# Coder-Yu/QRec

Hardware: NVIDIA H100
Metric: BPR triples/sec at d=64 (higher is better)
Workload: dtype f32

## Files before the change

include/qrec.h:

```cpp
#ifndef QREC_H_
#define QREC_H_

#include <stdint.h>

#ifdef __cplusplus
extern "C" {
#endif

#define QREC_OK 0
#define QREC_ERR_ARG (-1)
#define QREC_ERR_CUDA (-2)
#define QREC_ERR_STATE (-3)
#define QREC_ERR_NOMEM (-4)

const char* qrec_last_error(void);
const char* qrec_version(void);
int64_t qrec_launch_count(void);

typedef struct qrec_mt19937 {
  uint32_t mt[624];
  uint32_t index;
} qrec_mt19937;

int qrec_mt_seed(qrec_mt19937* st, uint64_t seed);
// ... 78 lines not shown

int qrec_bpr_sgd_batch_tma_f32(float* dev_P, float* dev_Q, int32_t d, int64_t n,
                               const int32_t* dev_u, const int32_t* dev_i, const int32_t* dev_j,
                               float lr, float reg_u, float reg_i, double* dev_loss, void* stream);

int qrec_bpr_sgd_usermajor_f32(float* dev_P, float* dev_Q, int32_t d, int32_t n_users, int64_t n, int32_t num_items,
                               const int64_t* dev_rowptr, const int32_t* dev_i, const int32_t* dev_j,
                               float lr, float reg_u, float reg_i, double* dev_loss, void* stream);

int qrec_bpr_epoch_usermajor_f32(float* dev_P, float* dev_Q, int32_t d, int32_t n_users, int64_t n,
                                 const int64_t* dev_rowptr, const int32_t* dev_i,
                                 const int64_t* dev_rated_rowptr, const int32_t* dev_rated_cols,
                                 int32_t num_items, uint64_t seed, uint32_t epoch, int32_t* dev_j_out,
                                 float lr, float reg_u, float reg_i, double* dev_loss, void* stream);

int qrec_rated_signature_build(int32_t n_users, const int64_t* dev_rated_rowptr, const int32_t* dev_rated_cols,
                               uint32_t* dev_sig, void* stream);
int qrec_bpr_epoch_usermajor_sig_f32(float* dev_P, float* dev_Q, int32_t d, int32_t n_users, int64_t n,
                                     const int64_t* dev_rowptr, const int32_t* dev_i,
                                     const int64_t* dev_rated_rowptr, const int32_t* dev_rated_cols,
                                     const uint32_t* dev_rated_sig, int32_t num_items, uint64_t seed,
                                     uint32_t epoch, int32_t* dev_j_out, float lr, float reg_u, float reg_i,
                                     double* dev_loss, void* stream);

int qrec_bpr_sgd_staged_f32(float* dev_P, int32_t d, int64_t n, const int32_t* dev_u,
                            const int32_t* dev_pos_i, const int32_t* dev_pos_j, const float* dev_R,
                            float* dev_D, float lr, float reg_u, float reg_i, double* dev_loss,
                            void* stream);

int qrec_sumsq_f32(const float* dev_x, int64_t n, double* dev_out, void* stream);
int qrec_sumsq_f64(const double* dev_x, int64_t n, double* dev_out, void* stream);

int qrec_table_snapshot_f32(const float* dev_src, float* dev_dst, int64_t n, void* stream);

int qrec_table_delta_f32(const float* dev_Q, const float* dev_B, float* dev_D, float* dev_S, int64_t n, void* stream);
int qrec_table_merge_f32(float* dev_Q, float* dev_B, const float* dev_D, const float* dev_S, int64_t n, void* stream);
int qrec_table_reduce_scatter_p2p_f32(const float* const* peer_D, int32_t world, int32_t rank, float* dev_S, int64_t n,
                                      void* stream);
int qrec_table_gather_merge_p2p_f32(const float* const* peer_S, int32_t world, float* dev_Q, float* dev_B,
                                    const float* dev_D, int64_t n, void* stream);

int qrec_score_topn_f32(const float* dev_U, const float* dev_V, int32_t d, int32_t n_items,
                        const int32_t* dev_user_ids, int32_t n_rows, const int64_t* dev_rated_rowptr,
                        const int32_t* dev_rated_cols, float rated_value, int32_t N, int32_t* dev_out_ids,
                        float* dev_out_scores, void* stream);
int qrec_score_topn_tc_f32(const float* dev_U, const float* dev_V, int32_t d, int32_t n_items,
                           const int32_t* dev_user_ids, int32_t n_rows, const int64_t* dev_rated_rowptr,
                           const int32_t* dev_rated_cols, float rated_value, int32_t N, int32_t* dev_out_ids,
                           float* dev_out_scores, void* stream);

int qrec_adj_normalize_f32(int32_t n_rows, const int64_t* dev_rowptr, const int32_t* dev_cols, const int32_t* dev_pair,
                           const float* dev_pair_w, float* dev_deg, float* dev_vals, void* stream);
int qrec_edge_keep_philox(int64_t n_lines, float drop_rate, uint64_t seed, uint32_t tag, uint32_t epoch,
                          uint8_t* dev_keep, void* stream);
int qrec_adj_line_weights_f32(int64_t n_lines, const int32_t* dev_line_pair, const uint8_t* dev_keep, int64_t n_pairs,
                              float* dev_pair_w, void* stream);
int qrec_adj_subgraph_count(int32_t n_rows, const int64_t* dev_rowptr, const int32_t* dev_pair, const float* dev_pair_w,
                            float* dev_deg, int64_t* dev_new_rowptr, int64_t* dev_scan_scratch, void* stream);
int qrec_adj_subgraph_fill_f32(int32_t n_rows, const int64_t* dev_rowptr, const int32_t* dev_cols, const int32_t* dev_pair,
                               const float* dev_pair_w, const float* dev_deg, const int64_t* dev_new_rowptr,
                               int32_t* dev_new_cols, float* dev_new_vals, void* stream);

int qrec_ubench_row_ops_f32(float* dev_table, int64_t rows, int64_t n_ops, int32_t mode, uint32_t seed,
                            float* dev_sink, void* stream);

typedef struct qrec_ctx qrec_ctx;
// ... 274 lines not shown
```

qrec_b200/_lib.py:

```python
import ctypes as C
import os

_HERE = os.path.dirname(os.path.abspath(__file__))
LIB_PATH = os.path.join(_HERE, 'libqrec.so')

c_i32p = C.POINTER(C.c_int32)
c_i64p = C.POINTER(C.c_int64)
c_u32p = C.POINTER(C.c_uint32)
c_u8p = C.POINTER(C.c_uint8)
c_f64p = C.POINTER(C.c_double)
vp = C.c_void_p


class MTState(C.Structure):
    _fields_ = [('mt', C.c_uint32 * 624), ('index', C.c_uint32)]


MTp = C.POINTER(MTState)

SIGNATURES = {
    'qrec_last_error': (C.c_char_p, []),
    'qrec_version': (C.c_char_p, []),
    'qrec_launch_count': (C.c_int64, []),
    'qrec_mt_seed': (C.c_int, [MTp, C.c_uint64]),
# ... 86 lines not shown
                                            vp, vp, vp, vp, C.c_int32, vp]),
    'qrec_svdpp_sgd_ordered_f64': (C.c_int, [vp, vp, vp, vp, vp, C.c_int32, C.c_int64, vp, vp, vp, vp, vp, C.c_double,
                                             C.c_double, C.c_double, C.c_double, C.c_double, C.c_double, vp, vp]),
    'qrec_svdpp_sgd_ordered_f32': (C.c_int, [vp, vp, vp, vp, vp, C.c_int32, C.c_int64, vp, vp, vp, vp, vp, C.c_float,
                                             C.c_float, C.c_float, C.c_float, C.c_float, C.c_float, vp, vp]),
    'qrec_svdpp_epoch_usermajor_f32': (C.c_int, [vp, vp, vp, vp, vp, C.c_int32, C.c_int32, vp, vp, vp, vp, C.c_float,
                                                 C.c_float, C.c_float, C.c_float, C.c_float, C.c_float, vp, C.c_int64,
                                                 vp]),
    'qrec_bpr_sgd_batch_f32': (C.c_int, [vp, vp, C.c_int32, C.c_int64, vp, vp, vp, C.c_float,
                                         C.c_float, C.c_float, vp, vp]),
    'qrec_bpr_sgd_batch_tma_f32': (C.c_int, [vp, vp, C.c_int32, C.c_int64, vp, vp, vp, C.c_float,
                                             C.c_float, C.c_float, vp, vp]),
    'qrec_bpr_sgd_usermajor_f32': (C.c_int, [vp, vp, C.c_int32, C.c_int32, C.c_int64, C.c_int32, vp, vp, vp, C.c_float,
                                             C.c_float, C.c_float, vp, vp]),
    'qrec_bpr_epoch_usermajor_f32': (C.c_int, [vp, vp, C.c_int32, C.c_int32, C.c_int64, vp, vp, vp, vp, C.c_int32,
                                               C.c_uint64, C.c_uint32, vp, C.c_float, C.c_float, C.c_float, vp, vp]),
    'qrec_bpr_sgd_staged_f32': (C.c_int, [vp, C.c_int32, C.c_int64, vp, vp, vp, vp, vp, C.c_float, C.c_float,
                                          C.c_float, vp, vp]),
    'qrec_ubench_row_ops_f32': (C.c_int, [vp, C.c_int64, C.c_int64, C.c_int32, C.c_uint32, vp, vp]),
    'qrec_table_delta_f32': (C.c_int, [vp, vp, vp, vp, C.c_int64, vp]),
    'qrec_table_merge_f32': (C.c_int, [vp, vp, vp, vp, C.c_int64, vp]),
    'qrec_table_reduce_scatter_p2p_f32': (C.c_int, [C.POINTER(vp), C.c_int32, C.c_int32, vp, C.c_int64, vp]),
    'qrec_table_gather_merge_p2p_f32': (C.c_int, [C.POINTER(vp), C.c_int32, vp, vp, vp, C.c_int64, vp]),
    'qrec_score_topn_f32': (C.c_int, [vp, vp, C.c_int32, C.c_int32, vp, C.c_int32, vp, vp, C.c_float, C.c_int32, vp, vp, vp]),
    'qrec_score_topn_tc_f32': (C.c_int, [vp, vp, C.c_int32, C.c_int32, vp, C.c_int32, vp, vp, C.c_float, C.c_int32, vp, vp, vp]),
    'qrec_adj_normalize_f32': (C.c_int, [C.c_int32, vp, vp, vp, vp, vp, vp, vp]),
    'qrec_edge_keep_philox': (C.c_int, [C.c_int64, C.c_float, C.c_uint64, C.c_uint32, C.c_uint32, vp, vp]),
    'qrec_adj_line_weights_f32': (C.c_int, [C.c_int64, vp, vp, C.c_int64, vp, vp]),
    'qrec_adj_subgraph_count': (C.c_int, [C.c_int32, vp, vp, vp, vp, vp, vp, vp]),
    'qrec_adj_subgraph_fill_f32': (C.c_int, [C.c_int32, vp, vp, vp, vp, vp, vp, vp, vp, vp]),
    'qrec_sumsq_f32': (C.c_int, [vp, C.c_int64, vp, vp]),
    'qrec_sumsq_f64': (C.c_int, [vp, C.c_int64, vp, vp]),
    'qrec_table_snapshot_f32': (C.c_int, [vp, vp, C.c_int64, vp]),
    'qrec_ctx_create': (C.c_int, [C.c_int, C.c_int64, C.POINTER(vp)]),
    'qrec_ctx_destroy': (C.c_int, [vp]),
    'qrec_ctx_set_rated_signature': (C.c_int, [vp, vp]),
    'qrec_bpr_epoch_host': (C.c_int, [vp, vp, vp, C.c_int32, C.c_int64, vp, vp, vp, C.c_float,
                                      C.c_float, C.c_float, c_f64p]),
    'qrec_bpr_epoch_usermajor_host': (C.c_int, [vp, vp, vp, C.c_int32, C.c_int32, vp, vp, vp, vp, C.c_int32, C.c_uint64,
                                                C.c_uint32, C.c_float, C.c_float, C.c_float, c_f64p]),
    'qrec_spmm_csr_f32': (C.c_int, [C.c_int32, C.c_int64, vp, vp, vp, vp, vp, C.c_int32, vp, C.c_float, vp]),
    'qrec_spmm_csr_rowsplit_f32': (C.c_int, [C.c_int32, C.c_int64, vp, vp, vp, vp, vp, C.c_int32, vp, C.c_float, vp]),
    'qrec_spmm_csr_scatter_rows_f32': (C.c_int, [C.c_int32, C.c_int32, vp, vp, vp, vp, vp, vp, C.c_int32, vp, C.c_float, vp]),
    'qrec_spmm_csr_rows_f32': (C.c_int, [C.c_int32, vp, vp, vp, vp, vp, vp, C.c_int32, C.c_int32, vp, C.c_float, vp]),
    'qrec_bpr_grad_scatter_f32': (C.c_int, [vp, vp, C.c_int32, C.c_int64, vp, vp, vp, C.c_float,
                                            C.c_float, vp, vp, vp, vp]),
    'qrec_bpr_grad_scatter_scaled_f32': (C.c_int, [vp, vp, C.c_int32, C.c_int64, vp, vp, vp, vp, C.c_float,
                                                   C.c_float, vp, vp, vp, vp]),
    'qrec_bpr_partial_scores_f32': (C.c_int, [vp, vp, C.c_int32, C.c_int64, vp, vp, vp, C.c_float, vp, vp, vp]),
    'qrec_bpr_grad_from_scores_f32': (C.c_int, [vp, vp, C.c_int32, C.c_int64, vp, vp, vp, vp, C.c_float, C.c_float, C.c_float, vp, vp, vp, vp]),
    'qrec_adam_dense_tf1_f32': (C.c_int, [vp, vp, vp, vp, C.c_int64, C.c_float, C.c_float,
                                          C.c_float, C.c_float, C.c_int64, vp]),
    'qrec_adam_dense_tf1_devstep_f32': (C.c_int, [vp, vp, vp, vp, C.c_int64, vp, C.c_float, C.c_float, C.c_float, vp]),
    'qrec_axpby_f32': (C.c_int, [vp, vp, vp, C.c_float, C.c_float, C.c_int64, vp]),
    'qrec_simgcl_perturb_f32': (C.c_int, [vp, C.c_int64, C.c_int32, C.c_int32, C.c_float, C.c_uint64, C.c_uint32,
                                          C.c_uint32, vp, C.c_float, vp]),
    'qrec_simgcl_perturb_rows_f32': (C.c_int, [vp, C.c_int64, C.c_int64, C.c_int32, C.c_int32, C.c_float, C.c_uint64, C.c_uint32,
                                               C.c_uint32, vp, C.c_float, vp]),
    'qrec_simgcl_perturb_listed_f32': (C.c_int, [vp, vp, C.c_int64, C.c_int64, C.c_int32, C.c_int32, C.c_float, C.c_uint64, C.c_uint32,
                                                  C.c_uint32, vp, C.c_float, vp]),
    'qrec_gather_normalize_f32': (C.c_int, [vp, vp, C.c_int32, C.c_int32, vp, vp, vp]),
    'qrec_infonce_rows_f32': (C.c_int, [vp, C.c_int32, C.c_float, vp, vp]),
    'qrec_normalize_bwd_scatter_f32': (C.c_int, [vp, vp, vp, vp, C.c_int32, C.c_int32, C.c_float, vp, vp]),
    'qrec_sgemm_f32': (C.c_int, [C.c_int32, C.c_int32, C.c_int32, C.c_int32, C.c_int32, C.c_float, vp,
                                 C.c_int32, vp, C.c_int32, C.c_float, vp, C.c_int32, vp]),
    'qrec_ngcf_act_fwd_f32': (C.c_int, [vp, C.c_int64, C.c_int32, C.c_float, C.c_int32, C.c_uint64,
# ... 47 lines not shown
```

qrec_b200/csrc/bpr_kernels.cu:

```cuda
#include <cmath>

#include "common.h"
#include "device.cuh"
#include "lane_shape.h"
#include "philox.cuh"
#include "bpr_step.cuh"
#include "um_waves.cuh"

namespace {

using namespace qrec;
using namespace qrec::bpr;

template <typename T, int E>
__global__ void __launch_bounds__(256)
bpr_sgd_ordered_kernel(T* __restrict__ P, T* __restrict__ Q, int d, long long n,
                       const int* __restrict__ u, const int* __restrict__ i,
                       const int* __restrict__ j, const int* __restrict__ wu,
                       const int* __restrict__ wi, const int* __restrict__ wj, int* ver_p,
                       int* ver_q, unsigned long long* ticket, T lr, T reg_u, T reg_i,
                       double* loss) {
  const int lane = threadIdx.x & 31;
  double local_loss = 0.0;
  const T a_u = mul_rn(lr, reg_u), a_i = mul_rn(lr, reg_i);
// ... 233 lines not shown
          float* trip = slot + (size_t)(r * TPW + sub) * ROWS * D;
          if (TMA_MASK & 1) *reinterpret_cast<float4*>(trip + SLOT_P * D + l * 4) = dp;
          else red_add_v4(P + (size_t)uu[r] * D + l * 4, dp);
          if (TMA_MASK & 2) *reinterpret_cast<float4*>(trip + SLOT_I * D + l * 4) = dqi;
          else red_add_v4(Q + (size_t)ii[r] * D + l * 4, dqi);
          if (TMA_MASK & 4) *reinterpret_cast<float4*>(trip + SLOT_J * D + l * 4) = dqj;
          else red_add_v4(Q + (size_t)jj[r] * D + l * 4, dqj);
        }
      }
      asm volatile("fence.proxy.async.shared::cta;" ::: "memory");
      __syncwarp();
      if (l < 3 && ((TMA_MASK >> l) & 1)) {
        const int srow = (l == 0) ? SLOT_P : (l == 1 ? SLOT_I : SLOT_J);
#pragma unroll
        for (int r = 0; r < UNROLL; ++r) {
          if (ok[r]) {
            float* dst = (l == 0) ? (P + (size_t)uu[r] * D) : (Q + (size_t)(l == 1 ? ii[r] : jj[r]) * D);
            const float* src = slot + (size_t)(r * TPW + sub) * ROWS * D + srow * D;
            asm volatile("cp.reduce.async.bulk.global.shared::cta.bulk_group.add.f32 [%0], [%1], %2;" ::"l"(dst),
                         "r"((uint32_t)__cvta_generic_to_shared(src)), "n"(D * 4)
                         : "memory");
          }
        }
        asm volatile("cp.async.bulk.commit_group;" ::: "memory");
      }
      buf ^= 1;
    }
  }
  if (l < 3) asm volatile("cp.async.bulk.wait_group 0;" ::: "memory");
  block_add_loss(lsum, loss);
}


template <int LPR, int G, bool FULL, bool SAMPLE, int MINB = 3, bool SIG = false>
__global__ void __launch_bounds__(256, MINB)
bpr_sgd_usermajor_kernel(float* __restrict__ P, float* __restrict__ Q, const float* __restrict__ Qr, int nvec, long long n,
                         const int* __restrict__ wave_user, const long long* __restrict__ rowptr,
                         const int* __restrict__ i, const int* __restrict__ j, float lr, float reg_u, float reg_i,
                         double* loss, FusedSampler fs, long long trip_off, const uint32_t* __restrict__ rated_sig) {
  constexpr int GPW = 32 / LPR;
  const int lane = threadIdx.x & 31;
  const int sub = lane / LPR, l = lane % LPR;
  const unsigned gmask = (LPR == 32) ? 0xffffffffu : (((1u << LPR) - 1u) << (sub * LPR));
  const int group = (int)((blockIdx.x * blockDim.x + threadIdx.x) >> 5) * GPW + sub;
  const int ngroups = (int)((gridDim.x * blockDim.x) >> 5) * GPW;
  const int d = FULL ? LPR * 4 : nvec * 4;
  const bool act = FULL ? true : (l < nvec);
  const float a_u = lr * reg_u, a_i = lr * reg_i;
  const float one_m_au = 1.0f - a_u, one_m_ai = 1.0f - a_i;
  float lsum = 0.f;
  qrec::pdl_launch_dependents();
  bool waited = false;
  const int ub = __ldg(wave_user + 1);
  for (int uu = __ldg(wave_user) + group; uu < ub; uu += ngroups) {
    long long lo = __ldg(rowptr + uu) - trip_off, hi = __ldg(rowptr + uu + 1) - trip_off;
    lo = lo > 0 ? lo : 0;
    hi = hi < n ? hi : n;
    if (lo >= hi) continue;
    float* prow = P + (size_t)uu * d + l * 4;
    float4 p = act ? *reinterpret_cast<const float4*>(prow) : make_float4(0.f, 0.f, 0.f, 0.f);
    long long rated_lo = 0, rated_hi = 0;
    if (SAMPLE) {
      rated_lo = __ldg(fs.rated_rowptr + uu);
      rated_hi = __ldg(fs.rated_rowptr + uu + 1);
    }
    for (long long base = lo; base < hi; base += LPR) {
      const int m = (hi - base) < LPR ? (int)(hi - base) : LPR;
      int mj = 0, mi = 0;
      if (l < m) {
        mi = __ldg(i + base + l);
        if (SAMPLE) {
          if (SIG)
            mj = qrec::sample_negative_sig(base + l + trip_off, fs.epoch, fs.seed_lo, fs.seed_hi, fs.num_items,
                                           fs.rated_cols, rated_lo, rated_hi,
                                           rated_sig + (size_t)uu * qrec::RATED_SIG_WORDS);
          else
            mj = qrec::sample_negative(base + l + trip_off, fs.epoch, fs.seed_lo, fs.seed_hi, fs.num_items, fs.rated_cols,
                                       rated_lo, rated_hi);
        } else {
          mj = __ldg(j + base + l);
        }
      }
      if (!waited) {
        qrec::pdl_wait();
        waited = true;
      }
      if (SAMPLE && l < m && fs.j_out != nullptr) fs.j_out[base + l] = mj;
      for (int t0 = 0; t0 < m; t0 += G) {
        float4 qi[G], qj[G];
        int ri[G], rj[G];
#pragma unroll
        for (int f = 0; f < G; ++f) {
          ri[f] = __shfl_sync(gmask, mi, sub * LPR + ((t0 + f) & (LPR - 1)));
          rj[f] = __shfl_sync(gmask, mj, sub * LPR + ((t0 + f) & (LPR - 1)));
          if (t0 + f < m && act) {
            qi[f] = qrec::ldg_no_l1_v4(reinterpret_cast<const float4*>(Qr + (size_t)ri[f] * d + l * 4));
            qj[f] = qrec::ldg_no_l1_v4(reinterpret_cast<const float4*>(Qr + (size_t)rj[f] * d + l * 4));
          } else {
            qi[f] = qj[f] = make_float4(0.f, 0.f, 0.f, 0.f);
          }
        }
#pragma unroll
        for (int f = 0; f < G; ++f) {
          if (t0 + f < m) {
            float x = dot4(p, qi[f]) - dot4(p, qj[f]);
            x = group_sum<LPR>(x, gmask);
            const float s = fast_sigmoid(x);
            const float g = lr * (1.0f - s);
            if (l == 0) lsum += fast_neg_log(s);
            if (act) {
              float4 dqi, dqj;
              bpr_step4_inplace(p, qi[f], qj[f], g, one_m_au, g * one_m_ai, a_i, dqi, dqj);
              red_add_v4(Q + (size_t)ri[f] * d + l * 4, dqi);
              red_add_v4(Q + (size_t)rj[f] * d + l * 4, dqj);
            }
          }
        }
      }
    }
    if (act) {
      const float4 p0 = __ldcg(reinterpret_cast<const float4*>(prow));
      red_add_v4(prow, make_float4(p.x - p0.x, p.y - p0.y, p.z - p0.z, p.w - p0.w));
    }
  }
  if (!waited) qrec::pdl_wait();
  block_add_loss(lsum, loss);
}

using UserMajorKernel = decltype(&bpr_sgd_usermajor_kernel<16, 4, true, false>);

template <int LPR>
UserMajorKernel usermajor_kernel(int nvec, bool sample, bool sig) {
  if (nvec != LPR)
    return sample ? bpr_sgd_usermajor_kernel<LPR, 4, false, true> : bpr_sgd_usermajor_kernel<LPR, 4, false, false>;
  if (sig) return bpr_sgd_usermajor_kernel<LPR, 2, true, true, 4, true>;
  return sample ? bpr_sgd_usermajor_kernel<LPR, 2, true, true, 4> : bpr_sgd_usermajor_kernel<LPR, 4, true, false>;
}

constexpr int UM_SNAPSHOT_THREADS = 512, UM_SNAPSHOT_CTAS_PER_SM = 4;
__global__ void __launch_bounds__(UM_SNAPSHOT_THREADS, UM_SNAPSHOT_CTAS_PER_SM)
um_snapshot_kernel(const float4* __restrict__ Q, float4* __restrict__ Qr, long long n4) {
  const unsigned long long keep = qrec::l2_policy_evict_last();
  qrec::pdl_wait();
  qrec::pdl_launch_dependents();
  const long long stride = (long long)gridDim.x * blockDim.x;
  long long k = (long long)blockIdx.x * blockDim.x + threadIdx.x;
  for (; k + 3 * stride < n4; k += 4 * stride) {
    float4 v[4];
#pragma unroll
    for (int r = 0; r < 4; ++r) v[r] = qrec::ld_stream_v4(Q + k + r * stride, keep);
#pragma unroll
    for (int r = 0; r < 4; ++r) qrec::st_hint_v4(Qr + k + r * stride, v[r], keep);
  }
  for (; k < n4; k += stride) qrec::st_hint_v4(Qr + k, qrec::ld_stream_v4(Q + k, keep), keep);
}

__global__ void __launch_bounds__(256)
um_wave_table_kernel(const long long* __restrict__ rowptr, int n_users, long long n, long long trip_off,
                     long long wave_chunks, long long nwaves, int* __restrict__ wave_user) {
  const long long w = (long long)blockIdx.x * blockDim.x + threadIdx.x;
  if (w <= nwaves) wave_user[w] = um_wave_first_user(rowptr, n_users, n, trip_off, wave_chunks, w);
}

__global__ void __launch_bounds__(256)
rated_signature_kernel(int n_users, const long long* __restrict__ rowptr, const int* __restrict__ cols,
                       uint32_t* __restrict__ sig) {
  const int lane = threadIdx.x & 31;
  const long long warp = ((long long)blockIdx.x * blockDim.x + threadIdx.x) >> 5;
  const long long nwarps = ((long long)gridDim.x * blockDim.x) >> 5;
  for (long long uu = warp; uu < n_users; uu += nwarps) {
    const long long lo = __ldg(rowptr + uu), hi = __ldg(rowptr + uu + 1);
    for (long long e = lo + lane; e < hi; e += 32) {
      const int c = __ldg(cols + e);
      atomicOr(sig + (size_t)uu * qrec::RATED_SIG_WORDS + ((c >> 5) & (qrec::RATED_SIG_WORDS - 1)), 1u << (c & 31));
    }
  }
}

template <typename T>
__global__ void __launch_bounds__(256)
sumsq_kernel(const T* __restrict__ x, long long n, double* out) {
  double acc = 0.0;
  const long long tid = (long long)blockIdx.x * blockDim.x + threadIdx.x;
  const long long stride = (long long)gridDim.x * blockDim.x;
  if constexpr (sizeof(T) == 4) {
    const long long n4 = n >> 2;
    const float4* x4 = reinterpret_cast<const float4*>(x);
// ... 87 lines not shown

int qrec_bpr_sgd_batch_tma_f32(float* P, float* Q, int32_t d, int64_t n, const int32_t* u,
                               const int32_t* i, const int32_t* j, float lr, float reg_u,
                               float reg_i, double* loss, void* stream) {
  QREC_REQUIRE(P && Q && loss, "qrec_bpr_sgd_batch_tma_f32: null pointer");
  QREC_REQUIRE(d == 64, "qrec_bpr_sgd_batch_tma_f32: only d=64 (got %d); use qrec_bpr_sgd_batch_f32", d);
  QREC_REQUIRE(n >= 0, "qrec_bpr_sgd_batch_tma_f32: n < 0");
  if (n == 0) return QREC_OK;
  QREC_REQUIRE(u && i && j, "qrec_bpr_sgd_batch_tma_f32: null index pointer");
  constexpr int UN = 4, MASK = 1;
  constexpr int smem = 8 * 2 * UN * 2 * 64 * 4;
  QREC_CUDA(allow_dynamic_smem((const void*)bpr_sgd_batch_tma_kernel<UN, MASK>, smem));
  const int grid = capped_grid(((n + 31) / 32 + 7) / 8, 2);
  bpr_sgd_batch_tma_kernel<UN, MASK><<<grid, 256, smem, (cudaStream_t)stream>>>(P, Q, n, u, i, j, lr, reg_u, reg_i, loss);
  QREC_LAUNCH_CHECK();
  return QREC_OK;
}

}

namespace qrec {
int launch_usermajor(float* P, float* Q, int32_t d, int32_t n_users, int64_t n, const int64_t* rowptr,
                     const int32_t* i, const int32_t* j, float lr, float reg_u, float reg_i, double* loss,
                     bool sample, const int64_t* rated_rowptr, const int32_t* rated_cols, int32_t num_items,
                     uint64_t seed, uint32_t epoch, int32_t* j_out, long long trip_off, cudaStream_t st,
                     const uint32_t* rated_sig) {
  if (n <= 0) return QREC_OK;
  QREC_REQUIRE(num_items >= 1, "qrec user-major epoch: num_items=%d (the item table's rows) must be given", num_items);
  FusedSampler fs = {reinterpret_cast<const long long*>(rated_rowptr), rated_cols, num_items, (uint32_t)seed,
                     (uint32_t)(seed >> 32), epoch, j_out};
  const int nvec = d / 4;
  const int lpr = row_lpr(nvec);
  const bool sig = sample && rated_sig != nullptr;
  const UserMajorKernel kernel =
      with_row_shape<128>(nvec, [&](auto s) { return usermajor_kernel<decltype(s)::LPR>(nvec, sample, sig); });
  int occ = 3;
  if (cudaOccupancyMaxActiveBlocksPerMultiprocessor(&occ, kernel, 256, 0) != cudaSuccess || occ < 1) occ = 3;
  const long long per_block = 8 * (32 / lpr);
  const long long max_users = n < n_users ? n : n_users;
  const int grid = capped_grid((max_users + per_block - 1) / per_block, occ);
  const size_t q_bytes = (size_t)num_items * d * sizeof(float);
  const long long wave = um_wave_chunks(n, num_items, d);
  const long long nwaves = um_num_waves(n, wave);
  float* Qr = nullptr;
  int* wave_user = nullptr;
  QREC_CUDA(cudaMallocAsync(reinterpret_cast<void**>(&Qr), q_bytes, st));
  const int rc = [&]() -> int {
    QREC_CUDA(cudaMallocAsync(reinterpret_cast<void**>(&wave_user), sizeof(int) * (size_t)(nwaves + 1), st));
    um_wave_table_kernel<<<(unsigned)((nwaves + 256) / 256), 256, 0, st>>>(reinterpret_cast<const long long*>(rowptr), n_users,
                                                                          n, trip_off, wave, nwaves, wave_user);
    QREC_CUDA(cudaGetLastError());
    count_launch();
    cudaLaunchAttribute pdl;
    pdl.id = cudaLaunchAttributeProgrammaticStreamSerialization;
    pdl.val.programmaticStreamSerializationAllowed = 1;
    const auto launch = [&](auto* fn, dim3 g, dim3 b, bool chained, auto... args) {
      cudaLaunchConfig_t cfg = {};
      cfg.gridDim = g;
      cfg.blockDim = b;
      cfg.stream = st;
      cfg.attrs = chained ? &pdl : nullptr;
      cfg.numAttrs = chained ? 1 : 0;
      return cudaLaunchKernelEx(&cfg, fn, args...);
    };
    const long long n4 = (long long)(q_bytes / sizeof(float4));
    const int copy_grid = sm_count() * UM_SNAPSHOT_CTAS_PER_SM;
    for (long long w = 0; w < nwaves; ++w) {
      QREC_CUDA(launch(um_snapshot_kernel, dim3(copy_grid), dim3(UM_SNAPSHOT_THREADS), w > 0,
                       reinterpret_cast<const float4*>(Q), reinterpret_cast<float4*>(Qr), n4));
      count_launch();
      QREC_CUDA(launch(kernel, dim3(grid), dim3(256), true, P, Q, static_cast<const float*>(Qr), nvec,
                       (long long)n, static_cast<const int*>(wave_user + w), reinterpret_cast<const long long*>(rowptr), i, j,
                       lr, reg_u, reg_i, loss, fs, trip_off, rated_sig));
      if (w + 1 < nwaves) count_launch();
    }
    return QREC_OK;
  }();
  if (wave_user != nullptr) QREC_CUDA(cudaFreeAsync(wave_user, st));
  QREC_CUDA(cudaFreeAsync(Qr, st));
  if (rc != QREC_OK) return rc;
  QREC_LAUNCH_CHECK();
  return QREC_OK;
}
}

extern "C" {

int qrec_bpr_sgd_usermajor_f32(float* P, float* Q, int32_t d, int32_t n_users, int64_t n, int32_t num_items,
                               const int64_t* rowptr, const int32_t* i, const int32_t* j, float lr, float reg_u, float reg_i,
                               double* loss, void* stream) {
  QREC_REQUIRE(P && Q && loss, "qrec_bpr_sgd_usermajor_f32: null pointer");
  QREC_REQUIRE(d >= 4 && d <= 128 && (d % 4) == 0, "qrec_bpr_sgd_usermajor_f32: d=%d unsupported (multiple of 4, 4..128)", d);
  QREC_REQUIRE(n_users >= 0 && n >= 0, "qrec_bpr_sgd_usermajor_f32: negative size");
  if (n_users == 0 || n == 0) return QREC_OK;
  QREC_REQUIRE(rowptr && i && j, "qrec_bpr_sgd_usermajor_f32: null index pointer");
  return qrec::launch_usermajor(P, Q, d, n_users, n, rowptr, i, j, lr, reg_u, reg_i, loss, false, nullptr, nullptr, num_items,
                                0, 0, nullptr, 0, (cudaStream_t)stream, nullptr);
}

int qrec_bpr_epoch_usermajor_f32(float* P, float* Q, int32_t d, int32_t n_users, int64_t n, const int64_t* rowptr,
                                 const int32_t* i, const int64_t* rated_rowptr, const int32_t* rated_cols,
                                 int32_t num_items, uint64_t seed, uint32_t epoch, int32_t* j_out, float lr,
                                 float reg_u, float reg_i, double* loss, void* stream) {
  QREC_REQUIRE(P && Q && loss, "qrec_bpr_epoch_usermajor_f32: null pointer");
  QREC_REQUIRE(d >= 4 && d <= 128 && (d % 4) == 0, "qrec_bpr_epoch_usermajor_f32: d=%d unsupported (multiple of 4, 4..128)", d);
  QREC_REQUIRE(n_users >= 0 && n >= 0 && num_items >= 1, "qrec_bpr_epoch_usermajor_f32: bad size");
  if (n_users == 0 || n == 0) return QREC_OK;
  QREC_REQUIRE(rowptr && i && rated_rowptr && rated_cols, "qrec_bpr_epoch_usermajor_f32: null index pointer");
  return qrec::launch_usermajor(P, Q, d, n_users, n, rowptr, i, nullptr, lr, reg_u, reg_i, loss, true, rated_rowptr,
                                rated_cols, num_items, seed, epoch, j_out, 0, (cudaStream_t)stream, nullptr);
}

int qrec_rated_signature_build(int32_t n_users, const int64_t* rated_rowptr, const int32_t* rated_cols,
                               uint32_t* sig, void* stream) {
  QREC_REQUIRE(n_users >= 0, "qrec_rated_signature_build: n_users < 0");
  if (n_users == 0) return QREC_OK;
  QREC_REQUIRE(rated_rowptr && rated_cols && sig, "qrec_rated_signature_build: null pointer");
  cudaStream_t st = (cudaStream_t)stream;
  QREC_CUDA(cudaMemsetAsync(sig, 0, (size_t)n_users * qrec::RATED_SIG_WORDS * sizeof(uint32_t), st));
  rated_signature_kernel<<<capped_grid(((long long)n_users + 7) / 8, 8), 256, 0, st>>>(n_users, reinterpret_cast<const long long*>(rated_rowptr),
                                                     rated_cols, sig);
  QREC_LAUNCH_CHECK();
  return QREC_OK;
}

int qrec_bpr_epoch_usermajor_sig_f32(float* P, float* Q, int32_t d, int32_t n_users, int64_t n, const int64_t* rowptr,
                                     const int32_t* i, const int64_t* rated_rowptr, const int32_t* rated_cols,
                                     const uint32_t* rated_sig, int32_t num_items, uint64_t seed, uint32_t epoch,
                                     int32_t* j_out, float lr, float reg_u, float reg_i, double* loss, void* stream) {
  QREC_REQUIRE(P && Q && loss, "qrec_bpr_epoch_usermajor_sig_f32: null pointer");
  QREC_REQUIRE(d == 16 || d == 32 || d == 64 || d == 128,
               "qrec_bpr_epoch_usermajor_sig_f32: d=%d unsupported (16, 32, 64 or 128); use qrec_bpr_epoch_usermajor_f32", d);
  QREC_REQUIRE(n_users >= 0 && n >= 0 && num_items >= 1, "qrec_bpr_epoch_usermajor_sig_f32: bad size");
  if (n_users == 0 || n == 0) return QREC_OK;
  QREC_REQUIRE(rowptr && i && rated_rowptr && rated_cols && rated_sig, "qrec_bpr_epoch_usermajor_sig_f32: null index pointer");
  return qrec::launch_usermajor(P, Q, d, n_users, n, rowptr, i, nullptr, lr, reg_u, reg_i, loss, true, rated_rowptr,
                                rated_cols, num_items, seed, epoch, j_out, 0, (cudaStream_t)stream, rated_sig);
}

int qrec_bpr_sgd_staged_f32(float* P, int32_t d, int64_t n, const int32_t* u, const int32_t* pos_i,
                            const int32_t* pos_j, const float* R, float* D, float lr, float reg_u,
                            float reg_i, double* loss, void* stream) {
  QREC_REQUIRE(d >= 4 && d <= 128 && (d % 4) == 0, "qrec_bpr_sgd_staged_f32: d=%d unsupported (multiple of 4, 4..128)", d);
  QREC_REQUIRE(n >= 0, "qrec_bpr_sgd_staged_f32: n < 0");
  if (n == 0) return QREC_OK;
  QREC_REQUIRE(P && u && pos_i && pos_j && R && D && loss, "qrec_bpr_sgd_staged_f32: null pointer");
  const int nvec = d / 4;
  cudaStream_t st = (cudaStream_t)stream;
  with_row_shape<128>(nvec, [&](auto s) {
    constexpr int LPR = decltype(s)::LPR;
    const long long per_block = 8 * (32 / LPR);
    const int grid = capped_grid((n + per_block - 1) / per_block, 8);
    bpr_sgd_staged_kernel<LPR><<<grid, 256, 0, st>>>(P, nvec, n, u, pos_i, pos_j, R, D, lr, reg_u, reg_i, loss);
  });
  QREC_LAUNCH_CHECK();
  return QREC_OK;
}

int qrec_sumsq_f32(const float* x, int64_t n, double* out, void* stream) {
  QREC_REQUIRE(out && (x || n == 0) && n >= 0, "qrec_sumsq_f32: bad argument");
  if (n == 0) return QREC_OK;
  QREC_REQUIRE((reinterpret_cast<uintptr_t>(x) & 15) == 0, "qrec_sumsq_f32: x not 16-byte aligned");
  sumsq_kernel<float><<<capped_grid((n / 4 + 255) / 256 + 1, 8), 256, 0, (cudaStream_t)stream>>>(x, n, out);
  QREC_LAUNCH_CHECK();
  return QREC_OK;
}

int qrec_table_snapshot_f32(const float* src, float* dst, int64_t n, void* stream) {
  QREC_REQUIRE(n >= 0 && (n % 4) == 0, "qrec_table_snapshot_f32: n=%lld must be a multiple of 4", (long long)n);
  if (n == 0) return QREC_OK;
  QREC_REQUIRE(src && dst, "qrec_table_snapshot_f32: null pointer");
  QREC_REQUIRE(((reinterpret_cast<uintptr_t>(src) | reinterpret_cast<uintptr_t>(dst)) & 15) == 0,
               "qrec_table_snapshot_f32: src and dst must be 16-byte aligned");
  um_snapshot_kernel<<<sm_count() * UM_SNAPSHOT_CTAS_PER_SM, UM_SNAPSHOT_THREADS, 0, (cudaStream_t)stream>>>(reinterpret_cast<const float4*>(src),
                                                                                 reinterpret_cast<float4*>(dst), n / 4);
  QREC_LAUNCH_CHECK();
  return QREC_OK;
}

int qrec_sumsq_f64(const double* x, int64_t n, double* out, void* stream) {
  QREC_REQUIRE(out && (x || n == 0) && n >= 0, "qrec_sumsq_f64: bad argument");
  if (n == 0) return QREC_OK;
  sumsq_kernel<double><<<capped_grid((n + 255) / 256, 8), 256, 0, (cudaStream_t)stream>>>(x, n, out);
  QREC_LAUNCH_CHECK();
  return QREC_OK;
}

}
```

qrec_b200/csrc/device.cuh:

```cuda
#pragma once
#include <cstdint>

namespace qrec {

__device__ __forceinline__ void red_add_v4(float* addr, float4 v) {
  asm volatile("red.global.add.v4.f32 [%0], {%1, %2, %3, %4};" ::"l"(addr), "f"(v.x), "f"(v.y), "f"(v.z), "f"(v.w) : "memory");
}

__device__ __forceinline__ unsigned long long l2_policy_evict_last() {
  unsigned long long pol;
  asm volatile("createpolicy.fractional.L2::evict_last.b64 %0, 1.0;" : "=l"(pol));
  return pol;
}
__device__ __forceinline__ float4 ld_stream_v4(const float4* p, unsigned long long pol) {
  float4 v;
  asm volatile("ld.global.nc.L1::no_allocate.L2::cache_hint.v4.f32 {%0, %1, %2, %3}, [%4], %5;"
               : "=f"(v.x), "=f"(v.y), "=f"(v.z), "=f"(v.w) : "l"(p), "l"(pol));
  return v;
}
__device__ __forceinline__ void st_hint_v4(float4* p, float4 v, unsigned long long pol) {
  asm volatile("st.global.L2::cache_hint.v4.f32 [%0], {%1, %2, %3, %4}, %5;" ::"l"(p), "f"(v.x), "f"(v.y), "f"(v.z), "f"(v.w),
               "l"(pol) : "memory");
}
__device__ __forceinline__ float4 ldg_no_l1_v4(const float4* p) {
  float4 v;
  asm volatile("ld.global.nc.L1::no_allocate.v4.f32 {%0, %1, %2, %3}, [%4];"
               : "=f"(v.x), "=f"(v.y), "=f"(v.z), "=f"(v.w) : "l"(p));
  return v;
}

__device__ __forceinline__ void pdl_wait() { asm volatile("griddepcontrol.wait;" ::: "memory"); }
__device__ __forceinline__ void pdl_launch_dependents() { asm volatile("griddepcontrol.launch_dependents;" ::: "memory"); }

__device__ __forceinline__ float dot4(float4 a, float4 b) { return a.x * b.x + a.y * b.y + a.z * b.z + a.w * b.w; }

__device__ __forceinline__ void fma4(float4& acc, float s, float4 x) {
  acc.x = fmaf(s, x.x, acc.x); acc.y = fmaf(s, x.y, acc.y);
  acc.z = fmaf(s, x.z, acc.z); acc.w = fmaf(s, x.w, acc.w);
}

template <typename T>
__device__ __forceinline__ T warp_sum(T v) {
#pragma unroll
  for (int o = 16; o > 0; o >>= 1) v += __shfl_xor_sync(0xffffffffu, v, o);
  return v;
}

template <int LPR>
__device__ __forceinline__ float group_sum(float v, unsigned mask = 0xffffffffu) {
#pragma unroll
  for (int o = LPR / 2; o > 0; o >>= 1) v += __shfl_xor_sync(mask, v, o);
  return v;
}

__device__ __forceinline__ float fast_sigmoid(float x) { return __fdividef(1.0f, 1.0f + __expf(-x)); }
// ... 42 lines not shown
    if (t != 0.0) atomicAdd(loss, t);
  }
}

__device__ __forceinline__ uint32_t smem_u32(const void* p) { return (uint32_t)__cvta_generic_to_shared(p); }

__device__ __forceinline__ void mbar_init(uint64_t* bar, uint32_t count) {
  asm volatile("mbarrier.init.shared::cta.b64 [%0], %1;" ::"r"(smem_u32(bar)), "r"(count));
}
__device__ __forceinline__ void mbar_expect_tx(uint64_t* bar, uint32_t bytes) {
  asm volatile("mbarrier.arrive.expect_tx.shared::cta.b64 _, [%0], %1;" ::"r"(smem_u32(bar)), "r"(bytes) : "memory");
}
__device__ __forceinline__ void mbar_arrive(uint64_t* bar) {
  asm volatile("mbarrier.arrive.shared::cta.b64 _, [%0];" ::"r"(smem_u32(bar)) : "memory");
}
__device__ __forceinline__ bool mbar_try_wait(uint64_t* bar, uint32_t parity) {
  uint32_t ok;
  asm volatile(
      "{\n\t.reg .pred p;\n\t"
      "mbarrier.try_wait.parity.shared::cta.b64 p, [%1], %2;\n\t"
      "selp.u32 %0, 1, 0, p;\n\t}"
      : "=r"(ok)
      : "r"(smem_u32(bar)), "r"(parity)
      : "memory");
  return ok != 0;
}
__device__ __forceinline__ void mbar_wait(uint64_t* bar, uint32_t parity) {
  for (uint32_t spins = 0;; ++spins) {
    if (mbar_try_wait(bar, parity)) return;
    if (spins > (1u << 22)) __trap();
  }
}

}
```

qrec_b200/engine.py:

```python
import contextlib
import ctypes as C
import math

import numpy as np

from ._lib import lib, check, MTState, QRecError


def _i32p(a):
    return a.ctypes.data_as(C.POINTER(C.c_int32))


def _i64p(a):
    return a.ctypes.data_as(C.POINTER(C.c_int64))


def version():
    return lib.qrec_version().decode()


def launch_count():
    return int(lib.qrec_launch_count())


# ... 484 lines not shown
          'qrec_adj_subgraph_fill_f32')
    return new_rowptr, new_cols, new_vals


def bucket_requests(ids, rows_per_rank, world, cap, count, send, pos, overflow):
    torch = _torch()
    check(lib.qrec_bucket_requests(_dev(ids, torch.int32, 'ids'), ids.shape[0], int(rows_per_rank), int(world), int(cap),
                                   _dev(count, torch.int32, 'count'), _dev(send, torch.int32, 'send'), _dev(pos, torch.int32, 'pos'),
                                   _dev(overflow, torch.int32, 'overflow'), _stream()), 'qrec_bucket_requests')


def gemv_t(A, v, out, alpha=1.0, beta=0.0):
    torch = _torch()
    ptr, ld = _strided_rows(A, 'A')
    check(lib.qrec_gemv_t_f32(ptr, max(ld, A.shape[1]), A.shape[0], A.shape[1], _opt(v, torch.float32, 'v'),
                              float(alpha), float(beta), _dev(out, torch.float32, 'out'), _stream()), 'qrec_gemv_t_f32')
    return out


def sumsq(x, out):
    torch = _torch()
    fn, _ = _entry('qrec_sumsq', x.dtype)
    check(fn(_dev(x, x.dtype, 'x'), x.numel(), _dev(out, torch.float64, 'out'), _stream()), 'qrec_sumsq')
    return out


def table_snapshot(src, dst):
    torch = _torch()
    if src.numel() != dst.numel():
        raise QRecError('table_snapshot: src has %d elements, dst %d' % (src.numel(), dst.numel()))
    check(lib.qrec_table_snapshot_f32(_dev(src, torch.float32, 'src'), _dev(dst, torch.float32, 'dst'), src.numel(),
                                      _stream()), 'qrec_table_snapshot_f32')
    return dst


def _host_ptr(a, dtype_np, dtype_t, name):
    torch = _torch()
    if isinstance(a, np.ndarray):
        assert a.dtype == dtype_np and a.flags.c_contiguous, name
        return a.ctypes.data, a.shape[0]
    assert (not a.is_cuda) and a.dtype == dtype_t and a.is_contiguous(), name
    return a.data_ptr(), a.shape[0]


class HostPipeline(object):

    def __init__(self, device=0, chunk_triples=1 << 22):
        self._ctx = C.c_void_p()
        check(lib.qrec_ctx_create(int(device), int(chunk_triples), C.byref(self._ctx)), 'qrec_ctx_create')

    def set_rated_signature(self, sig):
        torch = _torch()
        self._sig = sig
        check(lib.qrec_ctx_set_rated_signature(self._ctx, _opt(sig, torch.int32, 'rated_sig')),
              'qrec_ctx_set_rated_signature')

    def close(self):
        if self._ctx:
            check(lib.qrec_ctx_destroy(self._ctx), 'qrec_ctx_destroy')
            self._ctx = C.c_void_p()

    def __del__(self):
        try:
            self.close()
        except Exception:
            pass
# ... 990 lines not shown
```

Before: 3.215 billion.

## Fuse per-wave Q snapshot copy into user-major BPR kernel via TMA bulk ring

Removes the separate snapshot kernel launched before each wave. Thread 0 of each BPR CTA now copies the Q table into the read-only replica Qr with cp.async.bulk through a 4-slot shared-memory ring, taking chunks from a global atomic counter. CTAs then spin on a release/acquire completion counter before starting the wave's updates. This saves one launch per wave and lets the copy overlap with sampling, but adds 32KB of dynamic shared memory per CTA, which can lower occupancy. It also adds a grid-wide spin wait that needs all CTAs to be co-resident.

```diff
diff --git a/include/qrec.h b/include/qrec.h
--- a/include/qrec.h
+++ b/include/qrec.h
@@ -134,6 +134,8 @@
 int qrec_sumsq_f64(const double* dev_x, int64_t n, double* dev_out, void* stream);
 
 int qrec_table_snapshot_f32(const float* dev_src, float* dev_dst, int64_t n, void* stream);
+
+int qrec_bpr_usermajor_ctas_per_sm(int32_t d, int32_t sample, int32_t sig, int32_t* out);
 
 int qrec_table_delta_f32(const float* dev_Q, const float* dev_B, float* dev_D, float* dev_S, int64_t n, void* stream);
 int qrec_table_merge_f32(float* dev_Q, float* dev_B, const float* dev_D, const float* dev_S, int64_t n, void* stream);
diff --git a/qrec_b200/_lib.py b/qrec_b200/_lib.py
--- a/qrec_b200/_lib.py
+++ b/qrec_b200/_lib.py
@@ -142,6 +142,7 @@
     'qrec_sumsq_f32': (C.c_int, [vp, C.c_int64, vp, vp]),
     'qrec_sumsq_f64': (C.c_int, [vp, C.c_int64, vp, vp]),
     'qrec_table_snapshot_f32': (C.c_int, [vp, vp, C.c_int64, vp]),
+    'qrec_bpr_usermajor_ctas_per_sm': (C.c_int, [C.c_int32, C.c_int32, C.c_int32, C.POINTER(C.c_int32)]),
     'qrec_ctx_create': (C.c_int, [C.c_int, C.c_int64, C.POINTER(vp)]),
     'qrec_ctx_destroy': (C.c_int, [vp]),
     'qrec_ctx_set_rated_signature': (C.c_int, [vp, vp]),
diff --git a/qrec_b200/csrc/bpr_kernels.cu b/qrec_b200/csrc/bpr_kernels.cu
--- a/qrec_b200/csrc/bpr_kernels.cu
+++ b/qrec_b200/csrc/bpr_kernels.cu
@@ -289,9 +289,63 @@
 }
 
 
+constexpr int UM_COPY_CHUNK = 8192, UM_COPY_SLOTS = 4;
+constexpr int UM_COPY_SMEM = UM_COPY_CHUNK * UM_COPY_SLOTS;
+
+extern __shared__ __align__(128) char um_ring[];
+
+__host__ __device__ inline long long um_copy_chunks(long long bytes) { return (bytes + UM_COPY_CHUNK - 1) / UM_COPY_CHUNK; }
+
+template <typename Next>
+__device__ __forceinline__ int copy_table_chunks(const char* src, char* dst, long long bytes, Next next) {
+  __shared__ uint64_t full[UM_COPY_SLOTS];
+  __shared__ long long held[UM_COPY_SLOTS];
+  const long long nchunks = um_copy_chunks(bytes);
+  const unsigned long long keep = qrec::l2_policy_evict_last();
+  for (int s = 0; s < UM_COPY_SLOTS; ++s) qrec::mbar_init(&full[s], 1);
+  asm volatile("fence.mbarrier_init.release.cluster;" ::: "memory");
+  asm volatile("fence.proxy.async.global;" ::: "memory");
+  const auto size = [&](long long c) { return (uint32_t)min((long long)UM_COPY_CHUNK, bytes - c * UM_COPY_CHUNK); };
+  const auto load = [&](int s, long long c) {
+    held[s] = c;
+    qrec::mbar_expect_tx(&full[s], size(c));
+    qrec::bulk_g2s_hint(um_ring + s * UM_COPY_CHUNK, src + c * UM_COPY_CHUNK, size(c), &full[s], keep);
+  };
+  int issued = 0, done = 0;
+  bool more = true;
+  for (; issued < UM_COPY_SLOTS; ++issued) {
+    const long long c = next();
+    if (c >= nchunks) {
+      more = false;
+      break;
+    }
+    load(issued, c);
+  }
+  for (; done < issued; ++done) {
+    const int s = done % UM_COPY_SLOTS;
+    qrec::mbar_wait(&full[s], (done / UM_COPY_SLOTS) & 1);
+    const long long c = held[s];
+    qrec::bulk_s2g_hint(dst + c * UM_COPY_CHUNK, um_ring + s * UM_COPY_CHUNK, size(c), keep);
+    asm volatile("cp.async.bulk.commit_group;" ::: "memory");
+    if (more) {
+      const long long next_c = next();
+      more = next_c < nchunks;
+      if (more) {
+        asm volatile("cp.async.bulk.wait_group.read 0;" ::: "memory");
+        load(s, next_c);
+        ++issued;
+      }
+    }
+  }
+  asm volatile("cp.async.bulk.wait_group 0;" ::: "memory");
+  asm volatile("fence.proxy.async.global;" ::: "memory");
+  return done;
+}
+
 template <int LPR, int G, bool FULL, bool SAMPLE, int MINB = 3, bool SIG = false>
 __global__ void __launch_bounds__(256, MINB)
-bpr_sgd_usermajor_kernel(float* __restrict__ P, float* __restrict__ Q, const float* __restrict__ Qr, int nvec, long long n,
+bpr_sgd_usermajor_kernel(float* __restrict__ P, float* __restrict__ Q, float* __restrict__ Qr, long long q_bytes,
+                         int* __restrict__ wave_sync, int nvec, long long n,
                          const int* __restrict__ wave_user, const long long* __restrict__ rowptr,
                          const int* __restrict__ i, const int* __restrict__ j, float lr, float reg_u, float reg_i,
                          double* loss, FusedSampler fs, long long trip_off, const uint32_t* __restrict__ rated_sig) {
@@ -307,6 +361,17 @@
   const float one_m_au = 1.0f - a_u, one_m_ai = 1.0f - a_i;
   float lsum = 0.f;
   qrec::pdl_launch_dependents();
+  const auto enter_wave = [&] {
+    qrec::pdl_wait();
+    if (threadIdx.x == 0) {
+      const int copied = copy_table_chunks(reinterpret_cast<const char*>(Q), reinterpret_cast<char*>(Qr), q_bytes,
+                                           [=] { return (long long)atomicAdd(wave_sync, 1); });
+      if (copied > 0) qrec::red_release_gpu_add(wave_sync + 1, copied);
+      const long long nchunks = um_copy_chunks(q_bytes);
+      qrec::spin_until<8, 64>([=] { return qrec::ld_acquire_gpu(wave_sync + 1) >= nchunks; });
+    }
+    asm volatile("barrier.sync 1;" ::: "memory");
+  };
   bool waited = false;
   const int ub = __ldg(wave_user + 1);
   for (int uu = __ldg(wave_user) + group; uu < ub; uu += ngroups) {
@@ -339,7 +404,7 @@
         }
       }
       if (!waited) {
-        qrec::pdl_wait();
+        enter_wave();
         waited = true;
       }
       if (SAMPLE && l < m && fs.j_out != nullptr) fs.j_out[base + l] = mj;
@@ -380,7 +445,7 @@
       red_add_v4(prow, make_float4(p.x - p0.x, p.y - p0.y, p.z - p0.z, p.w - p0.w));
     }
   }
-  if (!waited) qrec::pdl_wait();
+  if (!waited) enter_wave();
   block_add_loss(lsum, loss);
 }
 
@@ -394,22 +459,24 @@
   return sample ? bpr_sgd_usermajor_kernel<LPR, 2, true, true, 4> : bpr_sgd_usermajor_kernel<LPR, 4, true, false>;
 }
 
-constexpr int UM_SNAPSHOT_THREADS = 512, UM_SNAPSHOT_CTAS_PER_SM = 4;
-__global__ void __launch_bounds__(UM_SNAPSHOT_THREADS, UM_SNAPSHOT_CTAS_PER_SM)
-um_snapshot_kernel(const float4* __restrict__ Q, float4* __restrict__ Qr, long long n4) {
-  const unsigned long long keep = qrec::l2_policy_evict_last();
-  qrec::pdl_wait();
-  qrec::pdl_launch_dependents();
-  const long long stride = (long long)gridDim.x * blockDim.x;
-  long long k = (long long)blockIdx.x * blockDim.x + threadIdx.x;
-  for (; k + 3 * stride < n4; k += 4 * stride) {
-    float4 v[4];
-#pragma unroll
-    for (int r = 0; r < 4; ++r) v[r] = qrec::ld_stream_v4(Q + k + r * stride, keep);
-#pragma unroll
-    for (int r = 0; r < 4; ++r) qrec::st_hint_v4(Qr + k + r * stride, v[r], keep);
-  }
-  for (; k < n4; k += stride) qrec::st_hint_v4(Qr + k, qrec::ld_stream_v4(Q + k, keep), keep);
+UserMajorKernel usermajor_for(int d, bool sample, bool sig, int* ctas_per_sm) {
+  const int nvec = d / 4;
+  const UserMajorKernel kernel =
+      with_row_shape<128>(nvec, [&](auto s) { return usermajor_kernel<decltype(s)::LPR>(nvec, sample, sig); });
+  int occ = 3;
+  if (cudaOccupancyMaxActiveBlocksPerMultiprocessor(&occ, kernel, 256, UM_COPY_SMEM) != cudaSuccess || occ < 1) occ = 3;
+  *ctas_per_sm = occ;
+  return kernel;
+}
+
+__global__ void __launch_bounds__(32) table_copy_kernel(const char* __restrict__ src, char* __restrict__ dst, long long bytes) {
+  if (threadIdx.x != 0) return;
+  long long c = blockIdx.x;
+  copy_table_chunks(src, dst, bytes, [&] {
+    const long long k = c;
+    c += gridDim.x;
+    return k;
+  });
 }
 
 __global__ void __launch_bounds__(256)
@@ -563,10 +630,8 @@
   const int nvec = d / 4;
   const int lpr = row_lpr(nvec);
   const bool sig = sample && rated_sig != nullptr;
-  const UserMajorKernel kernel =
-      with_row_shape<128>(nvec, [&](auto s) { return usermajor_kernel<decltype(s)::LPR>(nvec, sample, sig); });
   int occ = 3;
-  if (cudaOccupancyMaxActiveBlocksPerMultiprocessor(&occ, kernel, 256, 0) != cudaSuccess || occ < 1) occ = 3;
+  const UserMajorKernel kernel = usermajor_for(d, sample, sig, &occ);
   const long long per_block = 8 * (32 / lpr);
   const long long max_users = n < n_users ? n : n_users;
   const int grid = capped_grid((max_users + per_block - 1) / per_block, occ);
@@ -577,7 +642,9 @@
   int* wave_user = nullptr;
   QREC_CUDA(cudaMallocAsync(reinterpret_cast<void**>(&Qr), q_bytes, st));
   const int rc = [&]() -> int {
-    QREC_CUDA(cudaMallocAsync(reinterpret_cast<void**>(&wave_user), sizeof(int) * (size_t)(nwaves + 1), st));
+    QREC_CUDA(cudaMallocAsync(reinterpret_cast<void**>(&wave_user), sizeof(int) * (size_t)(3 * nwaves + 1), st));
+    int* wave_sync = wave_user + nwaves + 1;
+    QREC_CUDA(cudaMemsetAsync(wave_sync, 0, sizeof(int) * (size_t)(2 * nwaves), st));
     um_wave_table_kernel<<<(unsigned)((nwaves + 256) / 256), 256, 0, st>>>(reinterpret_cast<const long long*>(rowptr), n_users,
                                                                           n, trip_off, wave, nwaves, wave_user);
     QREC_CUDA(cudaGetLastError());
@@ -585,24 +652,17 @@
     cudaLaunchAttribute pdl;
     pdl.id = cudaLaunchAttributeProgrammaticStreamSerialization;
     pdl.val.programmaticStreamSerializationAllowed = 1;
-    const auto launch = [&](auto* fn, dim3 g, dim3 b, bool chained, auto... args) {
+    for (long long w = 0; w < nwaves; ++w) {
       cudaLaunchConfig_t cfg = {};
-      cfg.gridDim = g;
-      cfg.blockDim = b;
+      cfg.gridDim = dim3(grid);
+      cfg.blockDim = dim3(256);
+      cfg.dynamicSmemBytes = UM_COPY_SMEM;
       cfg.stream = st;
-      cfg.attrs = chained ? &pdl : nullptr;
-      cfg.numAttrs = chained ? 1 : 0;
-      return cudaLaunchKernelEx(&cfg, fn, args...);
-    };
-    const long long n4 = (long long)(q_bytes / sizeof(float4));
-    const int copy_grid = sm_count() * UM_SNAPSHOT_CTAS_PER_SM;
-    for (long long w = 0; w < nwaves; ++w) {
-      QREC_CUDA(launch(um_snapshot_kernel, dim3(copy_grid), dim3(UM_SNAPSHOT_THREADS), w > 0,
-                       reinterpret_cast<const float4*>(Q), reinterpret_cast<float4*>(Qr), n4));
-      count_launch();
-      QREC_CUDA(launch(kernel, dim3(grid), dim3(256), true, P, Q, static_cast<const float*>(Qr), nvec,
-                       (long long)n, static_cast<const int*>(wave_user + w), reinterpret_cast<const long long*>(rowptr), i, j,
-                       lr, reg_u, reg_i, loss, fs, trip_off, rated_sig));
+      cfg.attrs = w > 0 ? &pdl : nullptr;
+      cfg.numAttrs = w > 0 ? 1 : 0;
+      QREC_CUDA(cudaLaunchKernelEx(&cfg, kernel, P, Q, Qr, (long long)q_bytes, wave_sync + 2 * w, nvec, (long long)n,
+                                   static_cast<const int*>(wave_user + w), reinterpret_cast<const long long*>(rowptr), i, j,
+                                   lr, reg_u, reg_i, loss, fs, trip_off, rated_sig));
       if (w + 1 < nwaves) count_launch();
     }
     return QREC_OK;
@@ -640,6 +700,15 @@
   QREC_REQUIRE(rowptr && i && rated_rowptr && rated_cols, "qrec_bpr_epoch_usermajor_f32: null index pointer");
   return qrec::launch_usermajor(P, Q, d, n_users, n, rowptr, i, nullptr, lr, reg_u, reg_i, loss, true, rated_rowptr,
                                 rated_cols, num_items, seed, epoch, j_out, 0, (cudaStream_t)stream, nullptr);
+}
+
+int qrec_bpr_usermajor_ctas_per_sm(int32_t d, int32_t sample, int32_t sig, int32_t* out) {
+  QREC_REQUIRE(out != nullptr, "qrec_bpr_usermajor_ctas_per_sm: null pointer");
+  QREC_REQUIRE(d >= 4 && d <= 128 && (d % 4) == 0, "qrec_bpr_usermajor_ctas_per_sm: d=%d unsupported (multiple of 4, 4..128)", d);
+  int occ = 0;
+  usermajor_for(d, sample != 0, sample != 0 && sig != 0, &occ);
+  *out = occ;
+  return QREC_OK;
 }
 
 int qrec_rated_signature_build(int32_t n_users, const int64_t* rated_rowptr, const int32_t* rated_cols,
@@ -703,8 +772,9 @@
   QREC_REQUIRE(src && dst, "qrec_table_snapshot_f32: null pointer");
   QREC_REQUIRE(((reinterpret_cast<uintptr_t>(src) | reinterpret_cast<uintptr_t>(dst)) & 15) == 0,
                "qrec_table_snapshot_f32: src and dst must be 16-byte aligned");
-  um_snapshot_kernel<<<sm_count() * UM_SNAPSHOT_CTAS_PER_SM, UM_SNAPSHOT_THREADS, 0, (cudaStream_t)stream>>>(reinterpret_cast<const float4*>(src),
-                                                                                 reinterpret_cast<float4*>(dst), n / 4);
+  const long long bytes = n * (long long)sizeof(float);
+  table_copy_kernel<<<capped_grid(um_copy_chunks(bytes), 4), 32, UM_COPY_SMEM, (cudaStream_t)stream>>>(
+      reinterpret_cast<const char*>(src), reinterpret_cast<char*>(dst), bytes);
   QREC_LAUNCH_CHECK();
   return QREC_OK;
 }
diff --git a/qrec_b200/csrc/device.cuh b/qrec_b200/csrc/device.cuh
--- a/qrec_b200/csrc/device.cuh
+++ b/qrec_b200/csrc/device.cuh
@@ -11,16 +11,6 @@
   unsigned long long pol;
   asm volatile("createpolicy.fractional.L2::evict_last.b64 %0, 1.0;" : "=l"(pol));
   return pol;
-}
-__device__ __forceinline__ float4 ld_stream_v4(const float4* p, unsigned long long pol) {
-  float4 v;
-  asm volatile("ld.global.nc.L1::no_allocate.L2::cache_hint.v4.f32 {%0, %1, %2, %3}, [%4], %5;"
-               : "=f"(v.x), "=f"(v.y), "=f"(v.z), "=f"(v.w) : "l"(p), "l"(pol));
-  return v;
-}
-__device__ __forceinline__ void st_hint_v4(float4* p, float4 v, unsigned long long pol) {
-  asm volatile("st.global.L2::cache_hint.v4.f32 [%0], {%1, %2, %3, %4}, %5;" ::"l"(p), "f"(v.x), "f"(v.y), "f"(v.z), "f"(v.w),
-               "l"(pol) : "memory");
 }
 __device__ __forceinline__ float4 ldg_no_l1_v4(const float4* p) {
   float4 v;
@@ -129,4 +119,14 @@
   }
 }
 
+__device__ __forceinline__ void bulk_g2s_hint(void* smem_dst, const void* gsrc, uint32_t bytes, uint64_t* bar,
+                                              unsigned long long pol) {
+  asm volatile("cp.async.bulk.shared::cluster.global.mbarrier::complete_tx::bytes.L2::cache_hint [%0], [%1], %2, [%3], %4;"
+               ::"r"(smem_u32(smem_dst)), "l"(gsrc), "r"(bytes), "r"(smem_u32(bar)), "l"(pol) : "memory");
 }
+__device__ __forceinline__ void bulk_s2g_hint(void* gdst, const void* smem_src, uint32_t bytes, unsigned long long pol) {
+  asm volatile("cp.async.bulk.global.shared::cta.bulk_group.L2::cache_hint [%0], [%1], %2, %3;"
+               ::"l"(gdst), "r"(smem_u32(smem_src)), "r"(bytes), "l"(pol) : "memory");
+}
+
+}
diff --git a/qrec_b200/engine.py b/qrec_b200/engine.py
--- a/qrec_b200/engine.py
+++ b/qrec_b200/engine.py
@@ -540,6 +540,13 @@
     check(lib.qrec_table_snapshot_f32(_dev(src, torch.float32, 'src'), _dev(dst, torch.float32, 'dst'), src.numel(),
                                       _stream()), 'qrec_table_snapshot_f32')
     return dst
+
+
+def usermajor_ctas_per_sm(d, sample=True, sig=True):
+    out = C.c_int32(0)
+    check(lib.qrec_bpr_usermajor_ctas_per_sm(int(d), int(bool(sample)), int(bool(sig)), C.byref(out)),
+          'qrec_bpr_usermajor_ctas_per_sm')
+    return out.value
 
 
 def _host_ptr(a, dtype_np, dtype_t, name):
```

After: 3.232 billion (median of 6 runs). No clear change (+0.5%).
